# ideafisher/ssUnet-GAN

Measured on AMD Instinct MI355X. Metric: train images/sec (512^2 tiles), higher is better.
Workload: dtype f32; 1 GPU; UNet_R_SS_v2 generator + SRGAN-style discriminator, one G+D step (train_seg_gan.py:182-233), 16 x 3x512x512 tiles per GPU, fp32, Adam lr 2e-5; global_batch=16, tile=512, parallelism=dp1, dead_d_param_grads_of_g_step=computed

## Files before the change

### ssunet-gan_amd/csrc/conv_args.h

```cpp
#pragma once
#include "common.h"

struct ConvArgs {
  const float* in1; const float* in2;
  const float* w; const float* bias; const float* res; float* out;
  double* bnpart;
  int C1, C2, ld1, ld2;
  int N, H, W;
  int Kp, kmode;
  int ldr, Cout, ldo;
  int GH, GW, OH, OW;
  int in_sy, in_sx, out_sy, out_sx, out_oy, out_ox;
  int ntaps;
  unsigned long long tap_bits;
  int act; float slope;
  int tiles_x, tiles_y, nsteps;
  int ntiles_n, xcd_swizzle;
  float* ws; int ksplit;
  int parity;
  const float* in_scale; const float* in_shift; int in_act; float in_slope;
  const float* bwd_x; int bwd_ldx; const float* bwd_scale; const float* bwd_shift; const float* bwd_mean; int bwd_act; float bwd_slope;
  const float* w32;
};


int ssg_conv_igemm_dma_launch(const ConvArgs& a, int variant, hipStream_t st);
int ssg_conv_dma_variant(const ConvArgs& a, int variant);

bool ssg_conv_halo_ok(const ConvArgs& a);
int ssg_conv_igemm_halo_launch(const ConvArgs& a, int variant, hipStream_t st);
int ssg_conv_halo_variant(const ConvArgs& a, int variant);
void ssg_conv_halo_tile(int halo_variant, int* th, int* tw, int* bn);
int ssg_conv_halo_ksplit(const ConvArgs& a, int variant);

bool ssg_conv_halo_x3_ok(const ConvArgs& a, int variant);
int ssg_conv_halo_x3_bn(const ConvArgs& a, int variant);
int ssg_conv_igemm_halo_x3_launch(const ConvArgs& a, int variant, hipStream_t st);
bool ssg_conv_halo_x3_parity_ok(const ConvArgs& a);
int ssg_conv_igemm_halo_x3_parity_launch(const ConvArgs& a, hipStream_t st);
int ssg_conv_halo_k32_fmt(const ConvArgs& a);
void ssg_conv_halo_k32_tile(int fmt, int* th, int* tw);
bool ssg_conv_halo_k32_in_affine_ok(const ConvArgs& a, int fmt);
bool ssg_conv_halo_k32_bwd_stats_ok(const ConvArgs& a, int fmt);
int ssg_conv_igemm_halo_k32_launch(const ConvArgs& a, int fmt, hipStream_t st);
int ssg_pack_split_k32_launch(const float* w_packed, int R, int Kp, int BN, void* out, hipStream_t st);
int ssg_conv_dma_x3_bn(const ConvArgs& a);
int ssg_conv_igemm_dma_x3_launch(const ConvArgs& a, hipStream_t st);

template <int BN, int WTN>
__device__ __forceinline__ void ssg_bnpart_put(float* lds_f, int j, float s1, float s2, float piv, int nv, int wm, int wn, int half, int l31) {
  double* red = (double*)lds_f;
  const double c = (double)piv, n = (double)nv;
  double d1 = (double)s1 + n * c;
  double d2 = (double)s2 + 2.0 * c * (double)s1 + n * c * c;
  d1 += __shfl_xor(d1, 32); d2 += __shfl_xor(d2, 32);
  if (half == 0) {
    red[(wm * 2 + 0) * BN + wn * WTN + j * 32 + l31] = d1;
    red[(wm * 2 + 1) * BN + wn * WTN + j * 32 + l31] = d2;
  }
}
__device__ __forceinline__ void ssg_bnpart_begin() { __syncthreads(); }
template <int NI, int WAVES_M, int BN, int WTN>
__device__ __forceinline__ void ssg_bnpart_finish(const ConvArgs& a, float* lds_f, int mtile, int n0, int wm, int wn, int half, int l31) {
  double* red = (double*)lds_f;
  __syncthreads();
  if (wm == 0 && half == 0) {
#pragma unroll
    for (int j = 0; j < NI; ++j) {
      const int col = wn * WTN + j * 32 + l31;
      const int co = n0 + col;
      if (co < a.Cout) {
        double t1 = 0, t2 = 0;
#pragma unroll
// ... 8 lines not shown
```

### ssunet-gan_amd/csrc/conv_igemm.hip

```cpp
#include "common.h"
#include "conv_thin.h"
#include "conv_args.h"
#include <stdlib.h>

#ifndef SSG_EXPERIMENT
#define SSG_EXPERIMENT 0
#endif

namespace {

constexpr int LDS_ROW = 20;

template <int BM, int BN, int WAVES_M, int WAVES_N>
__global__ __launch_bounds__(256) void conv_igemm_kernel(const ConvArgs a) {
  static_assert(WAVES_M * WAVES_N == 4, "4 waves per workgroup");
  constexpr int TH = BM / 16;
  constexpr int WTM = BM / WAVES_M, WTN = BN / WAVES_N;
  constexpr int MI = WTM / 32, NI = WTN / 32;
  constexpr int A_LD = BM * 4 / 256;
  constexpr int B_LD = (BN * 4 + 255) / 256;
  static_assert(MI >= 1 && NI >= 1, "wave tile");

  __shared__ __attribute__((aligned(16))) float lds[2 * (BM + BN) * LDS_ROW];
  float* As = lds;
// ... 221 lines not shown
  ConvArgs a;
  a.in1 = d->in1; a.in2 = d->C2 ? d->in2 : d->in1; a.w = d->w; a.bias = d->bias; a.res = d->res; a.out = d->out;
  a.bnpart = d->bnpart;
  a.C1 = d->C1; a.C2 = d->C2; a.ld1 = d->ld1; a.ld2 = d->C2 ? d->ld2 : d->ld1;
  a.N = d->N; a.H = d->H; a.W = d->W; a.Kp = d->Kp; a.kmode = d->kmode;
  a.ldr = d->ldr; a.Cout = d->Cout; a.ldo = d->ldo;
  a.GH = d->GH; a.GW = d->GW; a.OH = d->OH; a.OW = d->OW;
  a.in_sy = d->in_sy; a.in_sx = d->in_sx; a.out_sy = d->out_sy; a.out_sx = d->out_sx;
  a.out_oy = d->out_oy; a.out_ox = d->out_ox;
  a.ntaps = d->ntaps;
  a.tap_bits = 0;
  for (int t = 0; t < d->ntaps; ++t)
    a.tap_bits |= (unsigned long long)(((d->dy[t] + 2) & 7) | (((d->dx[t] + 2) & 7) << 3)) << (6 * t);
  a.act = d->act; a.slope = d->slope;
  a.nsteps = d->Kp / 16;
  a.tiles_x = a.tiles_y = 0;
  a.ws = nullptr; a.ksplit = 1;
  a.parity = d->parity_merge;
  a.w32 = d->w;
  a.in_scale = d->in_scale; a.in_shift = d->in_shift; a.in_act = d->in_act; a.in_slope = d->in_slope;
  a.bwd_x = d->bwd_x; a.bwd_ldx = d->bwd_ldx; a.bwd_scale = d->bwd_scale; a.bwd_shift = d->bwd_shift; a.bwd_mean = d->bwd_mean;
  a.bwd_act = d->bwd_act; a.bwd_slope = d->bwd_slope;
  return a;
}

int split_bn(const ssg_conv_desc* d) {
  if (d->Cout <= 32) {
    if (d->kmode != 0 || d->parity_merge) return 0;
    const ConvArgs a = to_args(d);
    return uses_halo(a) ? ssg_conv_halo_k32_fmt(a) : 0;
  }
  if (!uses_dma(d)) return 0;
  const ConvArgs a = to_args(d);
  if (d->parity_merge) return ssg_conv_halo_x3_parity_ok(a) ? 64 : 0;
  if (!uses_halo(a)) return ssg_conv_dma_x3_bn(a);
  if (!ssg_conv_halo_x3_ok(a, pick_variant(d))) return 0;
  const int k32 = ssg_conv_halo_k32_fmt(a);
  if (k32) return k32;
  if (d->ldo % 4 == 0 && !((uintptr_t)d->out & 15) && ssg_conv_halo_ksplit(a, pick_variant(d)) > 1) return 0;
  return ssg_conv_halo_x3_bn(a, pick_variant(d));
}


}

extern "C" int ssg_conv2d_bnpart_rows(const ssg_conv_desc* d) {
  if (!d || validate(d) != SSG_OK) return 0;
  if (ssg_thin4_conv_kind(d) || ssg_thin_conv_kind(d)) return 0;
  const bool narrow_k32 = d->Cout <= 32 && d->w_split && split_bn(d) >= 1000;
  if (!uses_dma(d) && !narrow_k32) return 0;
  const ConvArgs a = to_args(d);
  int th, tw;
  if (d->w_split && split_bn(d) > 0) {
    if (split_bn(d) >= 1000) ssg_conv_halo_k32_tile(split_bn(d), &th, &tw);
    else if (uses_halo(a)) { th = 4; tw = 32; } else { th = 8; tw = 16; }
  }
  else if (uses_halo(a)) {
    if (d->ldo % 4 == 0 && !((uintptr_t)d->out & 15) && ssg_conv_halo_ksplit(a, pick_variant(d)) > 1) return 0;
    int bn; ssg_conv_halo_tile(ssg_conv_halo_variant(a, pick_variant(d)), &th, &tw, &bn);
  }
  else { th = ssg_conv_dma_variant(a, pick_variant(d)) == 1 ? 16 : 8; tw = 16; }
  return ((d->GW + tw - 1) / tw) * ((d->GH + th - 1) / th) * d->N;
}

static int64_t splitk_bytes(const ssg_conv_desc* d, int* ksplit) {
  *ksplit = 1;
  if (!uses_dma(d)) return 0;
// ... 21 lines not shown

extern "C" int ssg_conv2d_bwd_stats_ok(const ssg_conv_desc* d) {
  if (!d || validate(d) != SSG_OK || !d->w_split || d->parity_merge || d->Cout <= 32 || d->res || d->bias || d->act != SSG_ACT_NONE || d->in_scale) return 0;
  if (ssg_thin4_conv_kind(d) || ssg_thin_conv_kind(d) || ssg_conv1x1_k64_ok(d)) return 0;
  const int fmt = split_bn(d);
  return fmt >= 1000 && ssg_conv_halo_k32_bwd_stats_ok(to_args(d), fmt) ? 1 : 0;
}

extern "C" int64_t ssg_conv2d_workspace_bytes(const ssg_conv_desc* d) {
  if (!d || validate(d) != SSG_OK || ssg_thin4_conv_kind(d) || ssg_thin_conv_kind(d)) return 0;
  int k;
  return splitk_bytes(d, &k);
}

extern "C" int ssg_conv2d_igemm_f32(const ssg_conv_desc* d, void* stream) {
  int rc = validate(d);
  if (rc != SSG_OK) return rc;
  SSG_REQUIRE(!d->in_scale || (d->in_shift && ssg_conv2d_in_affine_ok(d)), SSG_EINVAL,
              "conv: in_scale on a descriptor whose kernel has no fused input transform (ssg_conv2d_in_affine_ok == 0)");
  SSG_REQUIRE(!d->bwd_x || (d->bnpart && d->bwd_scale && d->bwd_shift && d->bwd_mean && ssg_conv2d_bwd_stats_ok(d)), SSG_EINVAL,
              "conv: bwd_x on a descriptor whose kernel has no backward-statistics epilogue (ssg_conv2d_bwd_stats_ok == 0), or without bnpart");
  ConvArgs a = to_args(d);
  hipStream_t st = (hipStream_t)stream;
  if (d->ws && !d->bnpart) {
    int k; const int64_t need = splitk_bytes(d, &k);
    if (need > 0 && d->ws_bytes >= need && !((uintptr_t)d->ws & 15)) { a.ws = d->ws; a.ksplit = k; }
  }
  if (d->Cout <= 32 && d->w_split && !d->parity_merge && split_bn(d) >= 1000) {
    SSG_REQUIRE(ssg_aligned16(d->w_split), SSG_EALIGN, "conv: w_split alignment");
    a.w = (const float*)d->w_split; a.ws = nullptr; a.ksplit = 1;
    return ssg_conv_igemm_halo_k32_launch(a, split_bn(d), st);
  }
  SSG_REQUIRE(!d->bnpart || uses_dma(d), SSG_EINVAL, "conv: bnpart given but this shape has no statistics epilogue (ssg_conv2d_bnpart_rows == 0)");
  SSG_REQUIRE(!d->parity_merge || (d->w_split && split_bn(d) == 64), SSG_EINVAL,
              "conv: parity_merge needs a descriptor for which ssg_conv2d_split_bn reports 64 and its w_split pack");
  if (uses_dma(d)) {
    if (d->w_split && split_bn(d) > 0) {
      SSG_REQUIRE(ssg_aligned16(d->w_split), SSG_EALIGN, "conv: w_split alignment");
      a.w = (const float*)d->w_split; a.ws = nullptr; a.ksplit = 1;
      if (d->parity_merge) return ssg_conv_igemm_halo_x3_parity_launch(a, st);
      if (!uses_halo(a)) return ssg_conv_igemm_dma_x3_launch(a, st);
      if (split_bn(d) >= 1000) return ssg_conv_igemm_halo_k32_launch(a, split_bn(d), st);
      return ssg_conv_igemm_halo_x3_launch(a, pick_variant(d), st);
    }
    if (uses_halo(a)) return ssg_conv_igemm_halo_launch(a, pick_variant(d), st);
    return ssg_conv_igemm_dma_launch(a, pick_variant(d), st);
  }
  switch (pick_variant(d)) {
    case 0: return launch<128, 128, 2, 2>(a, st);
    case 1: return launch<256, 64, 4, 1>(a, st);
    default: return launch<256, 32, 4, 1>(a, st);
  }
}

extern "C" int ssg_conv2d_kernel_id(const ssg_conv_desc* d) {
  if (!d) return SSG_EINVAL;
  const int k4 = ssg_thin4_conv_kind(d);
  if (k4) return ssg_thin4_conv_id(d, k4);
  const int k = ssg_thin_conv_kind(d);
  if (k) return 9 + k;
  if (ssg_conv1x1_k64_ok(d)) return 16;
  if (uses_dma(d)) return uses_halo(to_args(d)) ? 30 + ssg_conv_halo_variant(to_args(d), pick_variant(d)) : 20 + ssg_conv_dma_variant(to_args(d), pick_variant(d));
  return pick_variant(d);
}

extern "C" int ssg_conv2d_f32(const ssg_conv_desc* d, void* stream) {
  int rc = validate(d);
  if (rc != SSG_OK) return rc;
  SSG_REQUIRE(!d->in_scale || (d->in_shift && ssg_conv2d_in_affine_ok(d)), SSG_EINVAL,
              "conv: in_scale on a descriptor whose kernel has no fused input transform (ssg_conv2d_in_affine_ok == 0)");
  SSG_REQUIRE(!d->bwd_x || (d->bnpart && d->bwd_scale && d->bwd_shift && d->bwd_mean && ssg_conv2d_bwd_stats_ok(d)), SSG_EINVAL,
              "conv: bwd_x on a descriptor whose kernel has no backward-statistics epilogue (ssg_conv2d_bwd_stats_ok == 0), or without bnpart");
  SSG_REQUIRE(!d->parity_merge || ssg_conv2d_split_bn(d) == 64, SSG_EINVAL,
              "conv: parity_merge on a descriptor that has no merged-parity kernel (ssg_conv2d_split_bn != 64)");
  if (d->parity_merge) return ssg_conv2d_igemm_f32(d, stream);
  const int k4 = ssg_thin4_conv_kind(d);
  const int k = k4 ? 0 : ssg_thin_conv_kind(d);
  SSG_REQUIRE(!d->bnpart || !(k4 || k), SSG_EINVAL, "conv: bnpart given but this shape has no statistics epilogue (ssg_conv2d_bnpart_rows == 0)");
  if (k4) return ssg_thin4_conv_launch(d, k4, (hipStream_t)stream);
  if (k) return ssg_thin_conv_launch(d, k, (hipStream_t)stream);
  if (ssg_conv1x1_k64_ok(d)) return ssg_conv1x1_k64_launch(d, (hipStream_t)stream);
  return ssg_conv2d_igemm_f32(d, stream);
}
```

### ssunet-gan_amd/csrc/conv_igemm_halo_k32.hip

```cpp
#include "common.h"
#include "lds_dma.h"
#include "conv_args.h"
#include "mfma_split.h"
#include "conv_slow.h"
#include <stdlib.h>

namespace {

typedef unsigned u32x4 __attribute__((ext_vector_type(4)));

#ifdef SSG_K32_PROBE
constexpr int SSG_PROBE_SLOTS = 32;
__device__ unsigned long long* ssg_probe_buf_k32 = nullptr;
#define SSG_STAMP(i) do { if (ssg_probe_buf_k32 && tid == 0) { ssg_probe_buf_k32[SSG_PROBE_SLOTS * blockIdx.x + (i)] = __builtin_amdgcn_s_memtime(); \
                                                            if ((i) == 0 || (i) == 3) ssg_probe_buf_k32[SSG_PROBE_SLOTS * blockIdx.x + 4 + ((i) == 3)] = __builtin_amdgcn_s_memrealtime(); } } while (0)
#define SSG_PROBE_NOW(v) unsigned long long v = __builtin_amdgcn_s_memtime(); asm volatile("s_waitcnt lgkmcnt(0)" : "+s"(v) :: "memory")
#else
#define SSG_STAMP(i) do { } while (0)
#endif

constexpr int SSG_K32_XF_MAXC = 512;

template <int TH, int BN, int WAVES_M, int WAVES_N, bool XF = false, bool BWD = false>
__global__ __launch_bounds__(WAVES_M * WAVES_N * 64, (WAVES_M * WAVES_N == 8) ? 1 : 2) void conv_halo_k32_kernel(const ConvArgs a) {
  constexpr int NW = WAVES_M * WAVES_N;
  constexpr int TW = 32, BM = TH * TW;
  constexpr int HW = TW + 2, HR = (TH + 2) * HW;
  constexpr int NPIX = (HR + 15) / 16 * 16;
  constexpr int KGS = NPIX * 16 + 64;
  constexpr int PLANE = 4 * KGS;
  constexpr int IMG = (3 * PLANE + 1023) / 1024 * 1024;
  constexpr int BSTG = BN * 192;
  constexpr int BPIECES = BSTG / 1024;
  constexpr int B_PC = (BPIECES + NW - 1) / NW;
  constexpr int WTM = BM / WAVES_M, WTN = BN / WAVES_N;
  constexpr int MI = WTM / 16, NI = WTN / 16;
  constexpr int NGRP = (HR + 7) / 8, GPW = (NGRP + NW - 1) / NW, NLD = GPW;
  constexpr int LD_T = 4;
  static_assert(IMG % 1024 == 0, "the ring behind the image stays 1-KiB aligned");
  static_assert(WTM == 64, "a wave owns two 32-pixel tile rows");

  extern __shared__ __attribute__((aligned(1024))) unsigned char lds[];
  unsigned char* const img = lds;
  unsigned char* const ring = lds + IMG;
  unsigned char* const ldsDummy = ring + 3 * BSTG;
  float* const xtab = (float*)(ldsDummy + 1024);

  const int tid = threadIdx.x, lane = tid & 63;
  const int wave = __builtin_amdgcn_readfirstlane(tid >> 6);
  const int wm = wave / WAVES_N, wn = wave % WAVES_N;
  const int l15 = lane & 15, kg = lane >> 4;

  SSG_STAMP(7);
  int bid = blockIdx.x;
  if (a.xcd_swizzle) {
    const int per = (int)gridDim.x >> 3;
    if (bid < per * 8) bid = (bid & 7) * per + (bid >> 3);
  }
  const int nyt = a.ntiles_n;
  const int nt = bid % nyt; bid /= nyt;
  const int n0 = nt * BN;
  const int tx = bid % a.tiles_x; bid /= a.tiles_x;
  const int ty = bid % a.tiles_y;
  const int n = bid / a.tiles_y;

  const int nchunks = (a.C1 + a.C2) >> 5;
  const int nsteps = nchunks * 9;
  const unsigned OOB = 0xffffffffu;
  const unsigned npix = (unsigned)a.N * (unsigned)a.H * (unsigned)a.W;
  const auto in1_rs = __builtin_amdgcn_make_buffer_rsrc(const_cast<float*>(a.in1), 0, (int)(npix * (unsigned)a.ld1 * 4u), 0x00020000);
  const auto in2_rs = __builtin_amdgcn_make_buffer_rsrc(const_cast<float*>(a.in2), 0, (int)(npix * (unsigned)a.ld2 * 4u), 0x00020000);
  const auto w_rs = __builtin_amdgcn_make_buffer_rsrc(const_cast<float*>(a.w), 0, (int)((unsigned)nyt * (unsigned)nsteps * (unsigned)BSTG), 0x00020000);
  const unsigned w_tile = (unsigned)nt * (unsigned)nsteps * (unsigned)BSTG;

  const int p8 = lane >> 3, q8 = lane & 7;
  const int hp0 = wave * GPW * 8 + p8;
  const int pix_base = (n * a.H + ty * TH - 1) * a.W + tx * TW - 1;
  auto px_pix_of = [&](int k) -> unsigned {
    const int hp = hp0 + 8 * k;
    const int hy = hp / HW, hx = hp - hy * HW;
    const bool ok = hp < HR && (unsigned)(ty * TH + hy - 1) < (unsigned)a.H && (unsigned)(tx * TW + hx - 1) < (unsigned)a.W;
    return ok ? (unsigned)(pix_base + hy * a.W + hx) : OOB;
  };
  const int px_dst0 = (q8 >> 1) * KGS + hp0 * 16 + (q8 & 1) * 8;
  u32x4 raw[NLD];
  auto load_px = [&](int chunk) {
    const int c0 = chunk * 32;
    const bool live = chunk < nchunks;
    const bool first = c0 < a.C1;
    const unsigned ld4 = (unsigned)(first ? a.ld1 : a.ld2) * 4u;
    const unsigned so = (unsigned)(first ? c0 : c0 - a.C1) * 4u;
#pragma unroll
    for (int k = 0; k < GPW; ++k) {
      const unsigned pix = px_pix_of(k);
      const unsigned vo = (live && pix != OOB) ? pix * ld4 + (unsigned)q8 * 16u : OOB;
      if (first) raw[k] = __builtin_amdgcn_raw_buffer_load_b128(in1_rs, vo, so, 0);
      else raw[k] = __builtin_amdgcn_raw_buffer_load_b128(in2_rs, vo, so, 0);
    }
  };
  bf16x4 cv[GPW][3];
  auto convert_px = [&](int chunk) {
#pragma unroll
    for (int k = 0; k < GPW; ++k) {
      f32x4 v = __builtin_bit_cast(f32x4, raw[k]);
      if constexpr (XF) {
        const int cb = (chunk < nchunks ? chunk : nchunks - 1) * 32 + q8 * 4;
        v = v * *(const f32x4*)(xtab + cb) + *(const f32x4*)(xtab + a.C1 + cb);
#pragma unroll
        for (int e = 0; e < 4; ++e) v[e] = ssg_act(v[e], a.in_act, a.in_slope);
        if (px_pix_of(k) == OOB) v = f32x4{0.f, 0.f, 0.f, 0.f};
      }
      split3_4(v, cv[k][0], cv[k][1], cv[k][2]);
    }
  };
  auto write_px = [&]() {
#pragma unroll
    for (int k = 0; k < GPW; ++k) {
      if (hp0 + 8 * k < HR) {
#pragma unroll
        for (int pl = 0; pl < 3; ++pl) *(bf16x4*)(img + pl * PLANE + px_dst0 + 128 * k) = cv[k][pl];
      }
    }
  };
  auto issue_b = [&](int s) {
    unsigned char* st = ring + (s % 3) * BSTG;
    const unsigned so = w_tile + (s < nsteps ? (unsigned)s * (unsigned)BSTG : 0u);
#pragma unroll
    for (int j = 0; j < B_PC; ++j) {
      const int g = wave + NW * j;
      if (BPIECES % NW == 0 || g < BPIECES) __builtin_amdgcn_raw_ptr_buffer_load_lds(w_rs, (ssg_lds_void*)(st + g * 1024), 16, (unsigned)lane * 16u, so + g * 1024, 0, 0);
      else __builtin_amdgcn_raw_ptr_buffer_load_lds(w_rs, (ssg_lds_void*)ldsDummy, 16, OOB, 0, 0, 0);
    }
  };

  f32x4 acc[MI][NI];
#pragma unroll
  for (int i = 0; i < MI; ++i)
#pragma unroll
    for (int j = 0; j < NI; ++j) acc[i][j] = f32x4{0.f, 0.f, 0.f, 0.f};

  int pb[MI];
#pragma unroll
  for (int i = 0; i < MI; ++i) {
    const int p = wm * WTM + i * 16 + l15;
    pb[i] = kg * KGS + (((p >> 5) + 1) * HW + (p & 31) + 1) * 16;
  }
  const int wfrag = wn * NI * 3 * 1024 + lane * 16;

  SSG_STAMP(0);
  load_px(0);
  issue_b(0);
  issue_b(1);
  if constexpr (XF) {
    for (int i = tid; i < 2 * a.C1; i += NW * 64) xtab[i] = i < a.C1 ? a.in_scale[i] : a.in_shift[i - a.C1];
    __syncthreads();
  }
  wait_vmcnt<2 * B_PC>();
  SSG_STAMP(6);
  convert_px(0);
  write_px();
  SSG_STAMP(1);

#ifdef SSG_K32_PROBE
  unsigned long long probe_own = 0, probe_bar = 0;
#endif
  for (int chunk = 0; chunk < nchunks; ++chunk) {
#pragma unroll
    for (int t = 0; t < 9; ++t) {
      const int s = chunk * 9 + t;
#ifndef SSG_K32_MIDBAR
#define SSG_K32_MIDBAR 0
#endif
#if SSG_K32_MIDBAR
      if (t == 0) {
        if (chunk > 0) write_px();
        wait_vmcnt<B_PC>();
        wait_lds_reads();
        __builtin_amdgcn_s_barrier();
        asm volatile("" ::: "memory");
      }
#else
#ifdef SSG_K32_PROBE
      SSG_PROBE_NOW(pb0);
#endif
      if (t == LD_T + 1 || t == LD_T + 2) wait_vmcnt<B_PC + NLD>();
      else wait_vmcnt<B_PC>();
      wait_lds_reads();
#ifdef SSG_K32_PROBE
      SSG_PROBE_NOW(pb1);
#endif
      __builtin_amdgcn_s_barrier();
      asm volatile("" ::: "memory");
#ifdef SSG_K32_PROBE
      SSG_PROBE_NOW(pb2);
      probe_own += pb1 - pb0; probe_bar += pb2 - pb1;
#endif
      if (t == 0 && chunk > 0) {
        write_px();
        wait_lds_reads();
        __builtin_amdgcn_s_barrier();
        asm volatile("" ::: "memory");
      }
#endif
#ifndef SSG_K32_DMA_MID
#define SSG_K32_DMA_MID 1
#endif
      constexpr bool MID = SSG_K32_DMA_MID && TH != 16;
      if constexpr (!MID) {
        issue_b(s + 2);
        if (t == LD_T) load_px(chunk + 1);
      }

      const int tb = (int)((a.tap_bits >> (6 * t)) & 63ull);
      const int toff = (((tb & 7) - 2) * HW + ((tb >> 3) - 2)) * 16;
      const unsigned char* st = ring + (t % 3) * BSTG + wfrag;
      bf16x8 p[MI][3], w[NI][3];
#ifndef SSG_K32_READ_ORDER
#define SSG_K32_READ_ORDER 0
#endif
#if SSG_K32_READ_ORDER
#pragma unroll
      for (int r = 0; r < 3; ++r) {
        const int qp = r, qw = 2 - r;
#pragma unroll
        for (int i = 0; i < MI; ++i) p[i][qp] = *(const bf16x8*)(img + qp * PLANE + pb[i] + toff);
#pragma unroll
        for (int j = 0; j < NI; ++j) w[j][qw] = *(const bf16x8*)(st + (j * 3 + qw) * 1024);
      }
#else
#pragma unroll
      for (int i = 0; i < MI; ++i)
#pragma unroll
        for (int q = 0; q < 3; ++q) p[i][q] = *(const bf16x8*)(img + q * PLANE + pb[i] + toff);
#pragma unroll
      for (int j = 0; j < NI; ++j)
#pragma unroll
        for (int q = 0; q < 3; ++q) w[j][q] = *(const bf16x8*)(st + (j * 3 + q) * 1024);
#endif
#ifndef SSG_K32_DYNPRIO
#define SSG_K32_DYNPRIO 1
#endif
      if (SSG_K32_DYNPRIO) __builtin_amdgcn_s_setprio(3);
#define SSG_K32_TERM(QW, QP)                                                                      \
  _Pragma("unroll") for (int j = 0; j < NI; ++j)                                                  \
  _Pragma("unroll") for (int i = 0; i < MI; ++i)                                                  \
      acc[i][j] = __builtin_amdgcn_mfma_f32_16x16x32_bf16(w[j][QW], p[i][QP], acc[i][j], 0, 0, 0);
      SSG_K32_TERM(2, 0) SSG_K32_TERM(1, 1)
      if constexpr (MID) {
        __builtin_amdgcn_sched_barrier(0);
        issue_b(s + 2);
        if (t == LD_T) load_px(chunk + 1);
        __builtin_amdgcn_sched_barrier(0);
      }
      if (SSG_K32_DYNPRIO) __builtin_amdgcn_s_setprio(2);
      SSG_K32_TERM(0, 2)
#if SSG_K32_MIDBAR
      {
#ifdef SSG_K32_PROBE
        SSG_PROBE_NOW(pb0);
#endif
        if (t == LD_T || t == LD_T + 1) wait_vmcnt<B_PC + NLD>();
        else wait_vmcnt<B_PC>();
        wait_lds_reads();
#ifdef SSG_K32_PROBE
        SSG_PROBE_NOW(pb1);
#endif
        __builtin_amdgcn_s_barrier();
        asm volatile("" ::: "memory");
#ifdef SSG_K32_PROBE
        SSG_PROBE_NOW(pb2);
        probe_own += pb1 - pb0; probe_bar += pb2 - pb1;
#endif
      }
#endif
      if (SSG_K32_DYNPRIO) __builtin_amdgcn_s_setprio(1);
      SSG_K32_TERM(1, 0) SSG_K32_TERM(0, 1)
      if (SSG_K32_DYNPRIO) __builtin_amdgcn_s_setprio(0);
      SSG_K32_TERM(0, 0)
#undef SSG_K32_TERM
      if (t == 8) {
#ifndef SSG_K32_CVT_FREE
#define SSG_K32_CVT_FREE 1
#endif
        if (!(SSG_K32_CVT_FREE && TH == 8 && !XF)) __builtin_amdgcn_sched_barrier(0);
        convert_px(chunk + 1);
      }
    }
  }
  wait_vmcnt<0>();
  wait_lds_reads();
  SSG_STAMP(2);
#ifdef SSG_K32_PROBE
  if (ssg_probe_buf_k32 && lane == 0) {
    ssg_probe_buf_k32[SSG_PROBE_SLOTS * blockIdx.x + 8 + 2 * wave] = probe_own;
    ssg_probe_buf_k32[SSG_PROBE_SLOTS * blockIdx.x + 9 + 2 * wave] = probe_bar;
  }
#endif

  {
    bool bad = false;
#pragma unroll
    for (int i = 0; i < MI; ++i)
#pragma unroll
      for (int j = 0; j < NI; ++j)
#pragma unroll
        for (int r = 0; r < 4; ++r) bad |= ssg_nonfinite(acc[i][j][r]);
    if (__builtin_amdgcn_readfirstlane(__syncthreads_or(bad))) {
      float* scr = (float*)lds + tid;
      const ConvArgs* ap = (const ConvArgs*)__builtin_amdgcn_kernarg_segment_ptr();
      asm volatile("" : "+s"(ap));
      const ConvArgs& as = *ap;
      for (int e = 0; e < MI * NI * 4; ++e) {
        const int i = e / (NI * 4), j = (e >> 2) % NI, r = e & 3;
        const int p = wm * WTM + i * 16 + l15;
        const int co = n0 + wn * WTN + j * 16 + kg * 4 + r;
        scr[e * (NW * 64)] = co < as.Cout ? ssg_conv_slow_value<XF>(as, n, ty * TH + (p >> 5), tx * TW + (p & 31), co, 0, 9) : 0.f;
      }
#pragma unroll
      for (int i = 0; i < MI; ++i)
#pragma unroll
        for (int j = 0; j < NI; ++j)
#pragma unroll
          for (int r = 0; r < 4; ++r) acc[i][j][r] = scr[((i * NI + j) * 4 + r) * (NW * 64)];
    }
  }

  SSG_STAMP(24);
  const bool want_bn = a.bnpart != nullptr;
  if (want_bn) __syncthreads();
  double* const red = (double*)lds;
  size_t opix[MI]; bool pok[MI];
#pragma unroll
  for (int i = 0; i < MI; ++i) {
    const int p = wm * WTM + i * 16 + l15;
    const int gy = ty * TH + (p >> 5), gx = tx * TW + (p & 31);
    pok[i] = gy < a.GH && gx < a.GW;
    opix[i] = (size_t)(n * a.OH + gy * a.out_sy + a.out_oy) * a.OW + gx * a.out_sx + a.out_ox;
  }
  float nvl = 0.f;
#pragma unroll
  for (int i = 0; i < MI; ++i) nvl += pok[i] ? 1.f : 0.f;
  if (want_bn) {
    nvl = ssg_row16_sum(nvl);
  }
  f32x4 bx[BWD ? MI : 1][BWD ? NI : 1];
  if constexpr (BWD) {
#pragma unroll
    for (int j = 0; j < NI; ++j)
#pragma unroll
      for (int i = 0; i < MI; ++i) {
        bx[i][j] = f32x4{0.f, 0.f, 0.f, 0.f};
        if (pok[i]) bx[i][j] = *(const f32x4*)(a.bwd_x + opix[i] * a.bwd_ldx + n0 + wn * WTN + j * 16 + kg * 4);
      }
  }
#pragma unroll
  for (int j = 0; j < NI; ++j) {
    const int co = n0 + wn * WTN + j * 16 + kg * 4;
// ... 67 lines not shown
      for (int k = 0; k < WAVES_M; ++k) { t1 += red[(k * 2 + 0) * BN + tid]; t2 += red[(k * 2 + 1) * BN + tid]; }
      double* dst = a.bnpart + (size_t)((n * a.tiles_y + ty) * a.tiles_x + tx) * 2 * a.Cout;
      dst[n0 + tid] = t1; dst[a.Cout + n0 + tid] = t2;
    }
  }
#ifdef SSG_K32_PROBE
  SSG_STAMP(25);
  asm volatile("s_waitcnt vmcnt(0)" ::: "memory");
  SSG_STAMP(3);
#endif
}

__global__ __launch_bounds__(256) void pack_split_k32_kernel(const float* __restrict__ w, int R, int Kp, int BN, unsigned char* __restrict__ out) {
  const int nsteps = Kp >> 5;
  const long long total = (long long)((R + BN - 1) / BN) * BN * nsteps * 4;
  for (long long i = (long long)blockIdx.x * 256 + threadIdx.x; i < total; i += (long long)gridDim.x * 256) {
    const int g = (int)(i & 3);
    long long t = i >> 2;
    const int s = (int)(t % nsteps); t /= nsteps;
    const int row = (int)t;
    const int tile = row / BN, rl = row - tile * BN;
    const int chunk32 = s / 9, tap = s - chunk32 * 9;
    const int chunk16 = chunk32 * 2 + (g >> 1);
    const float* src = w + (size_t)row * Kp + (size_t)(chunk16 * 9 + tap) * 16 + (g & 1) * 8;
    bf16x8 p1, p2, p3;
    const f32x4 z = {0.f, 0.f, 0.f, 0.f};
    split3(row < R ? *(const f32x4*)src : z, row < R ? *(const f32x4*)(src + 4) : z, p1, p2, p3);
    const int j = rl >> 4, l = (rl & 15) + 16 * g;
    unsigned char* dst = out + ((size_t)tile * nsteps + s) * BN * 192 + (size_t)j * 3 * 1024 + (size_t)l * 16;
    *(bf16x8*)(dst) = p1; *(bf16x8*)(dst + 1024) = p2; *(bf16x8*)(dst + 2048) = p3;
  }
}

template <int TH, int BN, int WAVES_M, int WAVES_N, bool XF = false, bool BWD = false>
int launch(const ConvArgs& a0, hipStream_t st) {
  ConvArgs a = a0;
  constexpr int NW = WAVES_M * WAVES_N;
  constexpr int HR = (TH + 2) * 34, NPIX = (HR + 15) / 16 * 16;
  a.tiles_x = (a.GW + 31) / 32;
  a.tiles_y = (a.GH + TH - 1) / TH;
  static const int swz = [] { const char* e = getenv("SSG_XCD_SWIZZLE"); return e ? atoi(e) : 1; }();
  a.xcd_swizzle = swz;
  a.ntiles_n = (a.Cout + BN - 1) / BN;
  dim3 grid((unsigned)(a.tiles_x * a.tiles_y * a.N * a.ntiles_n));
  constexpr int lds_bytes = (3 * 4 * (NPIX * 16 + 64) + 1023) / 1024 * 1024 + 3 * BN * 192 + 1024;
  static_assert(lds_bytes <= 160 * 1024 && (NW != 4 || BN <= 32 || lds_bytes <= 80 * 1024), "LDS budget");
  constexpr int tab_bytes = XF ? 2 * SSG_K32_XF_MAXC * 4 : 0;
  static_assert(lds_bytes + tab_bytes <= 160 * 1024, "LDS budget with the input-transform table");
  static const hipError_t attr = hipFuncSetAttribute((const void*)conv_halo_k32_kernel<TH, BN, WAVES_M, WAVES_N, XF, BWD>,
                                                     hipFuncAttributeMaxDynamicSharedMemorySize, lds_bytes + tab_bytes);
  if (attr != hipSuccess) { ssg_set_error("conv halo k32: LDS attribute: %s", hipGetErrorString(attr)); return (int)attr; }
  hipLaunchKernelGGL((conv_halo_k32_kernel<TH, BN, WAVES_M, WAVES_N, XF, BWD>), grid, dim3(NW * 64), lds_bytes + (XF ? 2 * a.C1 * 4 : 0), st, a);
  SSG_LAUNCH_CHECK();
  return SSG_OK;
}

}

#ifdef SSG_K32_PROBE
extern "C" int ssg_debug_set_probe_buffer_k32(void* p) {
  unsigned long long* v = (unsigned long long*)p;
  return (int)hipMemcpyToSymbol(HIP_SYMBOL(ssg_probe_buf_k32), &v, sizeof(v));
}
#endif

static int g_k32_mode = -1;
extern "C" int ssg_conv_set_k32_mode(int mode) {
  SSG_REQUIRE(mode >= 0 && mode <= 2, SSG_EINVAL, "k32 mode %d", mode);
  g_k32_mode = mode;
  return SSG_OK;
}

int ssg_conv_halo_k32_fmt(const ConvArgs& a) {
  if (g_k32_mode < 0) { const char* e = getenv("SSG_K32"); g_k32_mode = e ? atoi(e) : 1; }
  const int on = g_k32_mode;
  if (!on || !ssg_conv_halo_ok(a) || a.parity) return 0;
  if ((a.C1 & 31) || (a.C2 & 31) || a.GW < 17) return 0;
  if ((a.ldo & 3) || ((uintptr_t)a.out & 15) || (a.res && ((a.ldr & 3) || ((uintptr_t)a.res & 15))) || (a.bias && ((uintptr_t)a.bias & 15))) return 0;
  const unsigned long long bytes = (unsigned long long)a.N * a.H * a.W * (unsigned long long)(a.ld1 > a.ld2 ? a.ld1 : a.ld2) * 4ull;
  if (bytes > 0xfffffff0ull) return 0;
  if (a.Cout <= 32) {
    static const int narrow = [] { const char* e = getenv("SSG_K32_NARROW"); return e ? atoi(e) : 1; }();
    const long long wgs = (long long)a.N * ((a.GH + 7) / 8) * ((a.GW + 31) / 32);
    if (!narrow || a.Cout < 12 || (a.Cout & 3) || a.C1 + a.C2 < 128) return 0;
    return (on == 2 || wgs >= 192) ? (a.Cout <= 16 ? 1016 : 1032) : 0;
  }
  if (a.Cout % 128 == 0) {
    const long long wgs = (long long)a.N * ((a.GH + 7) / 8) * ((a.GW + 31) / 32) * (a.Cout / 128);
    const long long waves = (wgs + 255) / 256;
    if (on == 2 || wgs >= 2048 || (wgs >= 256 && wgs * 10 >= waves * 256 * 8)) return 1128;
  }
  if (a.Cout % 64 == 0) {
    static const int t16 = [] { const char* e = getenv("SSG_K32_T16"); return e ? atoi(e) : 1; }();
    const long long wgs16 = (long long)a.N * ((a.GH + 15) / 16) * ((a.GW + 31) / 32) * (a.Cout / 64);
    if (t16 && !a.in_scale && a.GH >= 16 && (wgs16 >= 2048 || (on == 2 && a.GH % 16 == 0))) return 2064;
    const long long wgs = (long long)a.N * ((a.GH + 3) / 4) * ((a.GW + 31) / 32) * (a.Cout / 64);
    if (on == 2 || wgs >= 1536) return 1064;
  }
  return 0;
}

void ssg_conv_halo_k32_tile(int fmt, int* th, int* tw) { *tw = 32; *th = (fmt == 1128 || fmt == 1016 || fmt == 1032) ? 8 : (fmt == 2064 ? 16 : 4); }

bool ssg_conv_halo_k32_in_affine_ok(const ConvArgs& a, int fmt) {
  if (fmt != 1128 && fmt != 1064) return false;
  if (a.C2 != 0 || a.C1 > SSG_K32_XF_MAXC) return false;
  return a.in_act == SSG_ACT_NONE || a.in_act == SSG_ACT_RELU || a.in_act == SSG_ACT_LRELU;
}

bool ssg_conv_halo_k32_bwd_stats_ok(const ConvArgs& a, int fmt) {
  if (fmt != 1128 && fmt != 1064 && fmt != 2064) return false;
  if ((a.bwd_ldx & 3) || ((uintptr_t)a.bwd_x & 15) || ((uintptr_t)a.bwd_scale & 15) || ((uintptr_t)a.bwd_shift & 15) || ((uintptr_t)a.bwd_mean & 15)) return false;
  return a.bwd_act == SSG_ACT_NONE || a.bwd_act == SSG_ACT_RELU || a.bwd_act == SSG_ACT_LRELU;
}

int ssg_conv_igemm_halo_k32_launch(const ConvArgs& a, int fmt, hipStream_t st) {
  if (a.bwd_x) {
    if (!a.bnpart || a.in_scale || !ssg_conv_halo_k32_bwd_stats_ok(a, fmt)) { ssg_set_error("conv halo k32: bwd_x on a launch without the backward-statistics epilogue"); return SSG_EINVAL; }
    if (fmt == 1128) return launch<8, 128, 4, 2, false, true>(a, st);
    if (fmt == 1064) return launch<4, 64, 2, 2, false, true>(a, st);
    return launch<16, 64, 8, 1, false, true>(a, st);
  }
  if (a.in_scale) {
    if (!a.in_shift || !ssg_conv_halo_k32_in_affine_ok(a, fmt)) { ssg_set_error("conv halo k32: in_scale on a launch without the fused input transform"); return SSG_EINVAL; }
    if (fmt == 1128) return launch<8, 128, 4, 2, true>(a, st);
    return launch<4, 64, 2, 2, true>(a, st);
  }
  if (fmt == 1128) return launch<8, 128, 4, 2>(a, st);
  if (fmt == 1064) return launch<4, 64, 2, 2>(a, st);
  if (fmt == 2064) return launch<16, 64, 8, 1>(a, st);
  if (fmt == 1016) return launch<8, 16, 4, 1>(a, st);
  if (fmt == 1032) return launch<8, 32, 4, 1>(a, st);
  ssg_set_error("conv halo k32: unknown format %d", fmt);
  return SSG_EINVAL;
}

int ssg_pack_split_k32_launch(const float* w_packed, int R, int Kp, int BN, void* out, hipStream_t st) {
  const long long total = (long long)((R + BN - 1) / BN) * BN * (Kp >> 5) * 4;
  long long blocks = (total + 255) / 256;
  if (blocks > 8192) blocks = 8192;
  hipLaunchKernelGGL(pack_split_k32_kernel, dim3((unsigned)blocks), dim3(256), 0, st, w_packed, R, Kp, BN, (unsigned char*)out);
  SSG_LAUNCH_CHECK();
  return SSG_OK;
}
```

### ssunet-gan_amd/ops.py

```python
import ctypes as C
import math

import torch
import torch.distributed as dist

from . import _lib
from ._lib import ACT_LRELU, ACT_NONE, ACT_RELU, ConvDesc, WgradDesc, call, ptr, stream_ptr

__all__ = ['conv2d', 'batch_norm_act', 'max_pool2x2', 'max_pool2x2_skip', 'max_unpool2x2', 'upsample2x_bilinear', 'upsample2x_nearest',
           'spade_modulate', 'adaptive_avgpool_flat', 'linear', 'seg_loss', 'bce_with_logits_const', 'nan_to_zero_',
           'to_nhwc', 'new_nhwc', 'bump_weight_epoch', 'dwconv2d', 'swish', 'sigmoid', 'gaussian', 'mul', 'global_avgpool',
           'channel_scale', 'spectral_norm_weight', 'conv2d_sn']


def pad4(c):
    return (c + 3) // 4 * 4


def new_nhwc(n, c, h, w, device, ld=None, zero=False):
    ld = pad4(c) if ld is None else ld
    buf = (torch.zeros if zero else torch.empty)(n * h * w * ld, device=device, dtype=torch.float32)
    return torch.empty(0, device=device, dtype=torch.float32).set_(
        buf.untyped_storage(), 0, (n, c, h, w), (h * w * ld, 1, w * ld, ld))

# ... 203 lines not shown

_DECLINED = object()


def _conv_launch(x1, x2, wpk, kp, kmode, row0, cout, bias, res, act, slope, taps, n, h, w, gh, gw, oh, ow,
                 in_s, out_s, out_oy, out_ox, out, want_bn=False, tag=None, parity_merge=False, in_affine=None, bwd_stats=None):
    d = ConvDesc()
    d.in1 = x1.data_ptr(); d.C1 = pad4(x1.shape[1]); d.ld1 = _ld(x1)
    if x2 is not None:
        d.in2 = x2.data_ptr(); d.C2 = pad4(x2.shape[1]); d.ld2 = _ld(x2)
    else:
        d.in2 = None; d.C2 = 0; d.ld2 = 0
    d.N, d.H, d.W = n, h, w
    d.w = wpk.data_ptr() + row0 * kp * 4; d.Kp = kp; d.kmode = kmode
    d.bias = bias.data_ptr() if bias is not None else None
    if res is not None:
        d.res = res.data_ptr(); d.ldr = _ld(res)
    else:
        d.res = None; d.ldr = 0
    d.out = out.data_ptr(); d.Cout = cout; d.ldo = _ld(out)
    d.GH, d.GW, d.OH, d.OW = gh, gw, oh, ow
    d.in_sy = d.in_sx = in_s
    d.out_sy = d.out_sx = out_s
    d.out_oy, d.out_ox = out_oy, out_ox
    _fill_taps(d, taps)
    d.act = act; d.slope = slope
    d.bnpart = None
    d.ws = None; d.ws_bytes = 0
    d.w_split = None
    d.parity_merge = 1 if parity_merge else 0
    d.in_scale = None; d.in_shift = None; d.in_act = ACT_NONE; d.in_slope = 0.0
    d.bwd_x = None; d.bwd_ldx = 0; d.bwd_scale = None; d.bwd_shift = None; d.bwd_mean = None; d.bwd_act = ACT_NONE; d.bwd_slope = 0.0
    split = None
    if parity_merge and not (MFMA_SPLIT and kmode == 0 and call('ssg_conv2d_split_bn', C.byref(d)) == 64):
        return False
    if MFMA_SPLIT and kmode == 0:
        bn = call('ssg_conv2d_split_bn', C.byref(d))
        if bn:
            split = _split_pack(wpk, row0, cout, kp, 1064 if bn == 2064 else bn)
            d.w_split = split.data_ptr()
    if in_affine is not None:
        d.in_scale = in_affine[0].data_ptr(); d.in_shift = in_affine[1].data_ptr(); d.in_act = int(in_affine[2]); d.in_slope = float(in_affine[3])
        if split is None or not call('ssg_conv2d_in_affine_ok', C.byref(d)):
            return _DECLINED
        bn = call('ssg_conv2d_split_bn', C.byref(d))
    if bwd_stats is not None:
        bx, bst, bact, bslope = bwd_stats
        d.bwd_x = bx.data_ptr(); d.bwd_ldx = _ld(bx); d.bwd_scale = bst[2].data_ptr(); d.bwd_shift = bst[3].data_ptr()
        d.bwd_mean = bst[0].data_ptr(); d.bwd_act = int(bact); d.bwd_slope = float(bslope)
        if split is None or not call('ssg_conv2d_bwd_stats_ok', C.byref(d)):
            return _DECLINED
        want_bn = True
    part = None
    if want_bn and BN_EPILOGUE:
        rows = call('ssg_conv2d_bnpart_rows', C.byref(d))
        if rows > 0:
            part = torch.empty((rows, 2, cout), dtype=torch.float64, device=out.device)
            d.bnpart = part.data_ptr()
    if bwd_stats is not None and part is None:
        return _DECLINED
    ws = None
    if part is None and split is None:
        need = call('ssg_conv2d_workspace_bytes', C.byref(d))
        if need > 0:
            ws = _ws(need, out.device)
            d.ws = ws.data_ptr(); d.ws_bytes = need
    cred = x1.shape[1] + (x2.shape[1] if x2 is not None else 0)
    label = None
    if PROFILE is not None:
        label = _CONV_LABELS.get(call('ssg_conv2d_kernel_id', C.byref(d)), '?') + ('+splitk' if ws is not None else '')
        if parity_merge:
            label = 'conv_igemm_halo_x3_kernel<128,64,4,1,true>'
        elif split is not None and bn >= 1000:
            label = {1128: 'conv_halo_k32_kernel<8,128>', 1064: 'conv_halo_k32_kernel<4,64>', 2064: 'conv_halo_k32_kernel<16,64>',
                     1016: 'conv_halo_k32_kernel<8,16>', 1032: 'conv_halo_k32_kernel<8,32>'}[bn]
        elif split is not None:
            if 'halo' in label:
                label = label.replace('conv_igemm_halo_kernel', 'conv_igemm_halo_x3_kernel').replace('<256,64>', '<128,64>')
            else:
                label = 'conv_igemm_dma_x3_kernel<%d>' % bn
        if PROFILE_SHAPES:
            label += ' n%d %dx%d cin%d cout%d taps%d s%d/%d' % (n, gh, gw, cred, cout, len(taps), in_s, out_s)
    with _Timed(label, 2.0 * n * gh * gw * cout * cred * len(taps), tag):
        call('ssg_conv2d_f32', C.byref(d), stream_ptr())
    return part


import os as _os
BN_EPILOGUE = _os.environ.get('SSG_BN_EPILOGUE', '1') != '0'
MFMA_SPLIT = _os.environ.get('SSG_MFMA_SPLIT', '1') == '1'
BN_FUSE_INPUT = _os.environ.get('SSG_BN_FUSE_INPUT', '0') == '1'
PARITY_MERGE = _os.environ.get('SSG_PARITY_MERGE', '1') != '0'


def _split_pack(wpk, row0, rows, kp, bn):
    cache = wpk.__dict__.get('_ssg_split')
    if cache is None:
        cache = {}
        try:
            wpk._ssg_split = cache
        except Exception:
            pass
    key = (row0, rows, bn)
    hit = cache.get(key)
    if hit is None:
# ... 1168 lines not shown
```

Before: 85.53 images/sec.

## Add merged-parity variant of the k32 halo conv kernel for stride-2 input gradients

Adds a PAR template mode to the bf16-split k32 halo convolution kernel so that merged-parity (stride-2 transposed or input-gradient) convolutions can run on it instead of the x3 parity kernel. The mode keeps four accumulator sets, one per output parity class, uses a one-sided halo, and writes each class to its interleaved output positions. A heuristic based on workgroup count and wave fill picks it, and an env var can turn it off. In exchange it raises register pressure (four accumulator sets, occupancy 1) and adds a per-element slow fallback path for non-finite results.

```diff
diff --git a/ssunet-gan_amd/csrc/conv_args.h b/ssunet-gan_amd/csrc/conv_args.h
--- a/ssunet-gan_amd/csrc/conv_args.h
+++ b/ssunet-gan_amd/csrc/conv_args.h
@@ -39,6 +39,7 @@
 bool ssg_conv_halo_x3_parity_ok(const ConvArgs& a);
 int ssg_conv_igemm_halo_x3_parity_launch(const ConvArgs& a, hipStream_t st);
 int ssg_conv_halo_k32_fmt(const ConvArgs& a);
+int ssg_conv_halo_k32_parity_fmt(const ConvArgs& a);
 void ssg_conv_halo_k32_tile(int fmt, int* th, int* tw);
 bool ssg_conv_halo_k32_in_affine_ok(const ConvArgs& a, int fmt);
 bool ssg_conv_halo_k32_bwd_stats_ok(const ConvArgs& a, int fmt);
diff --git a/ssunet-gan_amd/csrc/conv_igemm.hip b/ssunet-gan_amd/csrc/conv_igemm.hip
--- a/ssunet-gan_amd/csrc/conv_igemm.hip
+++ b/ssunet-gan_amd/csrc/conv_igemm.hip
@@ -277,7 +277,11 @@
   }
   if (!uses_dma(d)) return 0;
   const ConvArgs a = to_args(d);
-  if (d->parity_merge) return ssg_conv_halo_x3_parity_ok(a) ? 64 : 0;
+  if (d->parity_merge) {
+    if (!ssg_conv_halo_x3_parity_ok(a)) return 0;
+    const int k32 = ssg_conv_halo_k32_parity_fmt(a);
+    return k32 ? k32 : 64;
+  }
   if (!uses_halo(a)) return ssg_conv_dma_x3_bn(a);
   if (!ssg_conv_halo_x3_ok(a, pick_variant(d))) return 0;
   const int k32 = ssg_conv_halo_k32_fmt(a);
@@ -365,13 +369,13 @@
     return ssg_conv_igemm_halo_k32_launch(a, split_bn(d), st);
   }
   SSG_REQUIRE(!d->bnpart || uses_dma(d), SSG_EINVAL, "conv: bnpart given but this shape has no statistics epilogue (ssg_conv2d_bnpart_rows == 0)");
-  SSG_REQUIRE(!d->parity_merge || (d->w_split && split_bn(d) == 64), SSG_EINVAL,
-              "conv: parity_merge needs a descriptor for which ssg_conv2d_split_bn reports 64 and its w_split pack");
+  SSG_REQUIRE(!d->parity_merge || (d->w_split && (split_bn(d) == 64 || split_bn(d) == 3064)), SSG_EINVAL,
+              "conv: parity_merge needs a descriptor for which ssg_conv2d_split_bn reports 64 or 3064 and its w_split pack");
   if (uses_dma(d)) {
     if (d->w_split && split_bn(d) > 0) {
       SSG_REQUIRE(ssg_aligned16(d->w_split), SSG_EALIGN, "conv: w_split alignment");
       a.w = (const float*)d->w_split; a.ws = nullptr; a.ksplit = 1;
-      if (d->parity_merge) return ssg_conv_igemm_halo_x3_parity_launch(a, st);
+      if (d->parity_merge) return split_bn(d) == 3064 ? ssg_conv_igemm_halo_k32_launch(a, 3064, st) : ssg_conv_igemm_halo_x3_parity_launch(a, st);
       if (!uses_halo(a)) return ssg_conv_igemm_dma_x3_launch(a, st);
       if (split_bn(d) >= 1000) return ssg_conv_igemm_halo_k32_launch(a, split_bn(d), st);
       return ssg_conv_igemm_halo_x3_launch(a, pick_variant(d), st);
@@ -404,8 +408,8 @@
               "conv: in_scale on a descriptor whose kernel has no fused input transform (ssg_conv2d_in_affine_ok == 0)");
   SSG_REQUIRE(!d->bwd_x || (d->bnpart && d->bwd_scale && d->bwd_shift && d->bwd_mean && ssg_conv2d_bwd_stats_ok(d)), SSG_EINVAL,
               "conv: bwd_x on a descriptor whose kernel has no backward-statistics epilogue (ssg_conv2d_bwd_stats_ok == 0), or without bnpart");
-  SSG_REQUIRE(!d->parity_merge || ssg_conv2d_split_bn(d) == 64, SSG_EINVAL,
-              "conv: parity_merge on a descriptor that has no merged-parity kernel (ssg_conv2d_split_bn != 64)");
+  SSG_REQUIRE(!d->parity_merge || ssg_conv2d_split_bn(d) == 64 || ssg_conv2d_split_bn(d) == 3064, SSG_EINVAL,
+              "conv: parity_merge on a descriptor that has no merged-parity kernel (ssg_conv2d_split_bn not 64 / 3064)");
   if (d->parity_merge) return ssg_conv2d_igemm_f32(d, stream);
   const int k4 = ssg_thin4_conv_kind(d);
   const int k = k4 ? 0 : ssg_thin_conv_kind(d);
diff --git a/ssunet-gan_amd/csrc/conv_igemm_halo_k32.hip b/ssunet-gan_amd/csrc/conv_igemm_halo_k32.hip
--- a/ssunet-gan_amd/csrc/conv_igemm_halo_k32.hip
+++ b/ssunet-gan_amd/csrc/conv_igemm_halo_k32.hip
@@ -21,11 +21,14 @@
 
 constexpr int SSG_K32_XF_MAXC = 512;
 
-template <int TH, int BN, int WAVES_M, int WAVES_N, bool XF = false, bool BWD = false>
-__global__ __launch_bounds__(WAVES_M * WAVES_N * 64, (WAVES_M * WAVES_N == 8) ? 1 : 2) void conv_halo_k32_kernel(const ConvArgs a) {
+template <int TH, int BN, int WAVES_M, int WAVES_N, bool XF = false, bool BWD = false, bool PAR = false>
+__global__ __launch_bounds__(WAVES_M * WAVES_N * 64, (WAVES_M * WAVES_N == 8 || PAR) ? 1 : 2) void conv_halo_k32_kernel(const ConvArgs a) {
   constexpr int NW = WAVES_M * WAVES_N;
+  constexpr int NCLS = PAR ? 4 : 1;
+  static_assert(!PAR || (TH == 8 && BN == 64 && WAVES_M == 4 && WAVES_N == 1 && !XF && !BWD), "the merged-parity tile is <8, 64> on 4 x 1 waves, plain epilogue");
   constexpr int TW = 32, BM = TH * TW;
-  constexpr int HW = TW + 2, HR = (TH + 2) * HW;
+  constexpr int HO = PAR ? 0 : 1;
+  constexpr int HW = TW + 1 + HO, HR = (TH + 1 + HO) * HW;
   constexpr int NPIX = (HR + 15) / 16 * 16;
   constexpr int KGS = NPIX * 16 + 64;
   constexpr int PLANE = 4 * KGS;
@@ -39,6 +42,7 @@
   constexpr int LD_T = 4;
   static_assert(IMG % 1024 == 0, "the ring behind the image stays 1-KiB aligned");
   static_assert(WTM == 64, "a wave owns two 32-pixel tile rows");
+  static_assert(!PAR || IMG >= NW * 4, "PAR: the workgroup OR of the non-finite check uses one word per wave of the dead image; its slow path uses no LDS");
 
   extern __shared__ __attribute__((aligned(1024))) unsigned char lds[];
   unsigned char* const img = lds;
@@ -75,11 +79,11 @@
 
   const int p8 = lane >> 3, q8 = lane & 7;
   const int hp0 = wave * GPW * 8 + p8;
-  const int pix_base = (n * a.H + ty * TH - 1) * a.W + tx * TW - 1;
+  const int pix_base = (n * a.H + ty * TH - HO) * a.W + tx * TW - HO;
   auto px_pix_of = [&](int k) -> unsigned {
     const int hp = hp0 + 8 * k;
     const int hy = hp / HW, hx = hp - hy * HW;
-    const bool ok = hp < HR && (unsigned)(ty * TH + hy - 1) < (unsigned)a.H && (unsigned)(tx * TW + hx - 1) < (unsigned)a.W;
+    const bool ok = hp < HR && (unsigned)(ty * TH + hy - HO) < (unsigned)a.H && (unsigned)(tx * TW + hx - HO) < (unsigned)a.W;
     return ok ? (unsigned)(pix_base + hy * a.W + hx) : OOB;
   };
   const int px_dst0 = (q8 >> 1) * KGS + hp0 * 16 + (q8 & 1) * 8;
@@ -133,17 +137,20 @@
     }
   };
 
-  f32x4 acc[MI][NI];
-#pragma unroll
-  for (int i = 0; i < MI; ++i)
-#pragma unroll
-    for (int j = 0; j < NI; ++j) acc[i][j] = f32x4{0.f, 0.f, 0.f, 0.f};
+  f32x4 accs[NCLS][MI][NI];
+  auto& acc = accs[0];
+#pragma unroll
+  for (int q = 0; q < NCLS; ++q)
+#pragma unroll
+    for (int i = 0; i < MI; ++i)
+#pragma unroll
+      for (int j = 0; j < NI; ++j) accs[q][i][j] = f32x4{0.f, 0.f, 0.f, 0.f};
 
   int pb[MI];
 #pragma unroll
   for (int i = 0; i < MI; ++i) {
     const int p = wm * WTM + i * 16 + l15;
-    pb[i] = kg * KGS + (((p >> 5) + 1) * HW + (p & 31) + 1) * 16;
+    pb[i] = kg * KGS + (((p >> 5) + HO) * HW + (p & 31) + HO) * 16;
   }
   const int wfrag = wn * NI * 3 * 1024 + lane * 16;
 
@@ -206,6 +213,7 @@
 #define SSG_K32_DMA_MID 1
 #endif
       constexpr bool MID = SSG_K32_DMA_MID && TH != 16;
+      const int cls = PAR ? (t < 1 ? 0 : (t < 3 ? 1 : (t < 5 ? 2 : 3))) : 0;
       if constexpr (!MID) {
         issue_b(s + 2);
         if (t == LD_T) load_px(chunk + 1);
@@ -244,7 +252,7 @@
 #define SSG_K32_TERM(QW, QP)                                                                      \
   _Pragma("unroll") for (int j = 0; j < NI; ++j)                                                  \
   _Pragma("unroll") for (int i = 0; i < MI; ++i)                                                  \
-      acc[i][j] = __builtin_amdgcn_mfma_f32_16x16x32_bf16(w[j][QW], p[i][QP], acc[i][j], 0, 0, 0);
+      accs[cls][i][j] = __builtin_amdgcn_mfma_f32_16x16x32_bf16(w[j][QW], p[i][QP], accs[cls][i][j], 0, 0, 0);
       SSG_K32_TERM(2, 0) SSG_K32_TERM(1, 1)
       if constexpr (MID) {
         __builtin_amdgcn_sched_barrier(0);
@@ -282,7 +290,7 @@
 #ifndef SSG_K32_CVT_FREE
 #define SSG_K32_CVT_FREE 1
 #endif
-        if (!(SSG_K32_CVT_FREE && TH == 8 && !XF)) __builtin_amdgcn_sched_barrier(0);
+        if (!(SSG_K32_CVT_FREE && TH == 8 && !XF && !PAR)) __builtin_amdgcn_sched_barrier(0);
         convert_px(chunk + 1);
       }
     }
@@ -300,12 +308,42 @@
   {
     bool bad = false;
 #pragma unroll
-    for (int i = 0; i < MI; ++i)
-#pragma unroll
-      for (int j = 0; j < NI; ++j)
-#pragma unroll
-        for (int r = 0; r < 4; ++r) bad |= ssg_nonfinite(acc[i][j][r]);
-    if (__builtin_amdgcn_readfirstlane(__syncthreads_or(bad))) {
+    for (int q = 0; q < NCLS; ++q)
+#pragma unroll
+      for (int i = 0; i < MI; ++i)
+#pragma unroll
+        for (int j = 0; j < NI; ++j)
+#pragma unroll
+          for (int r = 0; r < 4; ++r) bad |= ssg_nonfinite(accs[q][i][j][r]);
+    int any;
+    if constexpr (PAR) {
+      const int wbad = __builtin_amdgcn_ballot_w64(bad) != 0;
+      __syncthreads();
+      ((int*)img)[wave] = wbad;
+      __syncthreads();
+      const int* f = (const int*)img;
+      any = f[0] | f[1] | f[2] | f[3];
+    } else {
+      any = __syncthreads_or(bad);
+    }
+    if (__builtin_amdgcn_readfirstlane(any)) {
+      if constexpr (PAR) {
+        const ConvArgs& as = *ssg_reload_args<ConvArgs>();
+        const int el = (int)__builtin_amdgcn_mbcnt_hi(~0u, __builtin_amdgcn_mbcnt_lo(~0u, 0u));
+#pragma unroll 1
+        for (int e = 0; e < 4 * MI * NI * 4; ++e) {
+          const int q = e / (MI * NI * 4), i = (e / (NI * 4)) % MI, j = (e >> 2) % NI, r = e & 3;
+          const int t_lo = q == 0 ? 0 : (q == 1 ? 1 : (q == 2 ? 3 : 5)), t_hi = q == 0 ? 1 : (q == 1 ? 3 : (q == 2 ? 5 : 9));
+          const int p = wm * WTM + i * 16 + (el & 15);
+          const int gy = ty * TH + (p >> 5), gx = tx * TW + (p & 31), co = n0 + wn * WTN + j * 16 + (el >> 4) * 4 + r;
+          const int GHq = (as.OH - (q >> 1) + 1) >> 1, GWq = (as.OW - (q & 1) + 1) >> 1;
+          if (gy < GHq && gx < GWq && co < as.Cout) {
+            const float v = ssg_conv_slow_value(as, n, gy, gx, co, t_lo, t_hi);
+            as.out[((size_t)(n * as.OH + 2 * gy + (q >> 1)) * as.OW + 2 * gx + (q & 1)) * as.ldo + co] = v;
+          }
+        }
+        return;
+      } else {
       float* scr = (float*)lds + tid;
       const ConvArgs* ap = (const ConvArgs*)__builtin_amdgcn_kernarg_segment_ptr();
       asm volatile("" : "+s"(ap));
@@ -322,7 +360,26 @@
         for (int j = 0; j < NI; ++j)
 #pragma unroll
           for (int r = 0; r < 4; ++r) acc[i][j][r] = scr[((i * NI + j) * 4 + r) * (NW * 64)];
-    }
+      }
+    }
+  }
+  if constexpr (PAR) {
+    const ConvArgs& ae = *ssg_reload_args<ConvArgs>();
+    const int el = (int)__builtin_amdgcn_mbcnt_hi(~0u, __builtin_amdgcn_mbcnt_lo(~0u, 0u));
+#pragma unroll
+    for (int q = 0; q < 4; ++q) {
+      const int GHq = (ae.OH - (q >> 1) + 1) >> 1, GWq = (ae.OW - (q & 1) + 1) >> 1;
+#pragma unroll
+      for (int i = 0; i < MI; ++i) {
+        const int p = wm * WTM + i * 16 + (el & 15);
+        const int gy = ty * TH + (p >> 5), gx = tx * TW + (p & 31);
+        if (gy >= GHq || gx >= GWq) continue;
+        float* const o = ae.out + ((size_t)(n * ae.OH + 2 * gy + (q >> 1)) * ae.OW + 2 * gx + (q & 1)) * ae.ldo + n0 + (el >> 4) * 4;
+#pragma unroll
+        for (int j = 0; j < NI; ++j) *(f32x4*)(o + j * 16) = accs[q][i][j];
+      }
+    }
+    return;
   }
 
   SSG_STAMP(24);
@@ -456,11 +513,11 @@
   }
 }
 
-template <int TH, int BN, int WAVES_M, int WAVES_N, bool XF = false, bool BWD = false>
+template <int TH, int BN, int WAVES_M, int WAVES_N, bool XF = false, bool BWD = false, bool PAR = false>
 int launch(const ConvArgs& a0, hipStream_t st) {
   ConvArgs a = a0;
   constexpr int NW = WAVES_M * WAVES_N;
-  constexpr int HR = (TH + 2) * 34, NPIX = (HR + 15) / 16 * 16;
+  constexpr int HR = PAR ? (TH + 1) * 33 : (TH + 2) * 34, NPIX = (HR + 15) / 16 * 16;
   a.tiles_x = (a.GW + 31) / 32;
   a.tiles_y = (a.GH + TH - 1) / TH;
   static const int swz = [] { const char* e = getenv("SSG_XCD_SWIZZLE"); return e ? atoi(e) : 1; }();
@@ -468,13 +525,13 @@
   a.ntiles_n = (a.Cout + BN - 1) / BN;
   dim3 grid((unsigned)(a.tiles_x * a.tiles_y * a.N * a.ntiles_n));
   constexpr int lds_bytes = (3 * 4 * (NPIX * 16 + 64) + 1023) / 1024 * 1024 + 3 * BN * 192 + 1024;
-  static_assert(lds_bytes <= 160 * 1024 && (NW != 4 || BN <= 32 || lds_bytes <= 80 * 1024), "LDS budget");
+  static_assert(lds_bytes <= 160 * 1024 && (NW != 4 || BN <= 32 || PAR || lds_bytes <= 80 * 1024), "LDS budget");
   constexpr int tab_bytes = XF ? 2 * SSG_K32_XF_MAXC * 4 : 0;
   static_assert(lds_bytes + tab_bytes <= 160 * 1024, "LDS budget with the input-transform table");
-  static const hipError_t attr = hipFuncSetAttribute((const void*)conv_halo_k32_kernel<TH, BN, WAVES_M, WAVES_N, XF, BWD>,
+  static const hipError_t attr = hipFuncSetAttribute((const void*)conv_halo_k32_kernel<TH, BN, WAVES_M, WAVES_N, XF, BWD, PAR>,
                                                      hipFuncAttributeMaxDynamicSharedMemorySize, lds_bytes + tab_bytes);
   if (attr != hipSuccess) { ssg_set_error("conv halo k32: LDS attribute: %s", hipGetErrorString(attr)); return (int)attr; }
-  hipLaunchKernelGGL((conv_halo_k32_kernel<TH, BN, WAVES_M, WAVES_N, XF, BWD>), grid, dim3(NW * 64), lds_bytes + (XF ? 2 * a.C1 * 4 : 0), st, a);
+  hipLaunchKernelGGL((conv_halo_k32_kernel<TH, BN, WAVES_M, WAVES_N, XF, BWD, PAR>), grid, dim3(NW * 64), lds_bytes + (XF ? 2 * a.C1 * 4 : 0), st, a);
   SSG_LAUNCH_CHECK();
   return SSG_OK;
 }
@@ -524,7 +581,16 @@
   return 0;
 }
 
-void ssg_conv_halo_k32_tile(int fmt, int* th, int* tw) { *tw = 32; *th = (fmt == 1128 || fmt == 1016 || fmt == 1032) ? 8 : (fmt == 2064 ? 16 : 4); }
+int ssg_conv_halo_k32_parity_fmt(const ConvArgs& a) {
+  static const int on = [] { const char* e = getenv("SSG_K32_S2"); return e ? atoi(e) : 1; }();
+  if (!on || !ssg_conv_halo_x3_parity_ok(a)) return 0;
+  if ((a.C1 & 31) || a.C2 || a.act != SSG_ACT_NONE || (a.ldo & 3) || ((uintptr_t)a.out & 15)) return 0;
+  const long long wgs = (long long)a.N * ((a.GH + 7) / 8) * ((a.GW + 31) / 32) * (a.Cout / 64);
+  const long long waves = (wgs + 255) / 256;
+  return (wgs >= 256 && wgs * 10 >= waves * 256 * 8) ? 3064 : 0;
+}
+
+void ssg_conv_halo_k32_tile(int fmt, int* th, int* tw) { *tw = 32; *th = (fmt == 1128 || fmt == 1016 || fmt == 1032 || fmt == 3064) ? 8 : (fmt == 2064 ? 16 : 4); }
 
 bool ssg_conv_halo_k32_in_affine_ok(const ConvArgs& a, int fmt) {
   if (fmt != 1128 && fmt != 1064) return false;
@@ -539,6 +605,10 @@
 }
 
 int ssg_conv_igemm_halo_k32_launch(const ConvArgs& a, int fmt, hipStream_t st) {
+  if (fmt == 3064) {
+    if (!a.parity || a.bwd_x || a.in_scale || !ssg_conv_halo_k32_parity_fmt(a)) { ssg_set_error("conv halo k32: format 3064 on a launch that is not a merged-parity input gradient"); return SSG_EINVAL; }
+    return launch<8, 64, 4, 1, false, false, true>(a, st);
+  }
   if (a.bwd_x) {
     if (!a.bnpart || a.in_scale || !ssg_conv_halo_k32_bwd_stats_ok(a, fmt)) { ssg_set_error("conv halo k32: bwd_x on a launch without the backward-statistics epilogue"); return SSG_EINVAL; }
     if (fmt == 1128) return launch<8, 128, 4, 2, false, true>(a, st);
diff --git a/ssunet-gan_amd/ops.py b/ssunet-gan_amd/ops.py
--- a/ssunet-gan_amd/ops.py
+++ b/ssunet-gan_amd/ops.py
@@ -259,12 +259,12 @@
     d.in_scale = None; d.in_shift = None; d.in_act = ACT_NONE; d.in_slope = 0.0
     d.bwd_x = None; d.bwd_ldx = 0; d.bwd_scale = None; d.bwd_shift = None; d.bwd_mean = None; d.bwd_act = ACT_NONE; d.bwd_slope = 0.0
     split = None
-    if parity_merge and not (MFMA_SPLIT and kmode == 0 and call('ssg_conv2d_split_bn', C.byref(d)) == 64):
+    if parity_merge and not (MFMA_SPLIT and kmode == 0 and call('ssg_conv2d_split_bn', C.byref(d)) in (64, 3064)):
         return False
     if MFMA_SPLIT and kmode == 0:
         bn = call('ssg_conv2d_split_bn', C.byref(d))
         if bn:
-            split = _split_pack(wpk, row0, cout, kp, 1064 if bn == 2064 else bn)
+            split = _split_pack(wpk, row0, cout, kp, 1064 if bn in (2064, 3064) else bn)
             d.w_split = split.data_ptr()
     if in_affine is not None:
         d.in_scale = in_affine[0].data_ptr(); d.in_shift = in_affine[1].data_ptr(); d.in_act = int(in_affine[2]); d.in_slope = float(in_affine[3])
@@ -297,7 +297,7 @@
     if PROFILE is not None:
         label = _CONV_LABELS.get(call('ssg_conv2d_kernel_id', C.byref(d)), '?') + ('+splitk' if ws is not None else '')
         if parity_merge:
-            label = 'conv_igemm_halo_x3_kernel<128,64,4,1,true>'
+            label = 'conv_halo_k32_kernel<8,64,parity>' if bn == 3064 else 'conv_igemm_halo_x3_kernel<128,64,4,1,true>'
         elif split is not None and bn >= 1000:
             label = {1128: 'conv_halo_k32_kernel<8,128>', 1064: 'conv_halo_k32_kernel<4,64>', 2064: 'conv_halo_k32_kernel<16,64>',
                      1016: 'conv_halo_k32_kernel<8,16>', 1032: 'conv_halo_k32_kernel<8,32>'}[bn]
```

New measurement: 85.26 images/sec (median of 2 runs). Within noise of the previous version (-0.3%).
